# jkrasting/momlevel

Hardware: AMD Instinct MI355X
Metric: Mcells/s for fused Wright-EOS+steric at 1440×1080×75; % HBM roofline (higher is better)
Workload: dtype f64

## Files before the change

momlevel_amd/core.py:

```python

import numpy as np
import torch

from . import _lib, hostio
from ._lib import (
    DTYPE_F32,
    DTYPE_F32_UPCAST,
    DTYPE_F64,
    DTYPE_T32_S64,
    DTYPE_T64_S32,
    EOS_IDS,
    FUNC_IDS,
    P_FULL3D,
    P_FULL4D,
    P_SCALAR,
    P_ZPROF,
    MomlevelHipError,
)

F32_MODES = {"faithful": DTYPE_F32, "upcast": DTYPE_F32_UPCAST}
K1_TCHUNK = {"steric": 32, "held": 64}
ARITH_FLAGS = {"exact": 0, "fused": _lib.FLAG_FMA}


def arith_default(kernel="k0", dtype=None):
    import os

    mode = os.environ.get("MOMLEVEL_AMD_ARITH")
    if mode is None:
        return "fused" if kernel == "k1" else "exact"
    if mode not in ARITH_FLAGS:
        raise ValueError(f"MOMLEVEL_AMD_ARITH must be 'exact' or 'fused', got '{mode}'")
    return mode


def _arith_flag(arith, kernel="k0", dtype=None):
    if dtype in (DTYPE_T32_S64, DTYPE_T64_S32):
        if arith == "fused":
            raise ValueError("arith='fused' is not available for thetao / so of different dtypes")
        return 0
    if arith is None:
        arith = arith_default(kernel, dtype)
    try:
        return ARITH_FLAGS[arith]
    except KeyError:
        raise ValueError(f"arith must be 'exact' or 'fused', got '{arith}'") from None


def require_device():
    _lib.load()
    if not torch.cuda.is_available():
        raise MomlevelHipError(
            "no HIP device visible: momlevel_amd computes on MI355X only (no CPU fallback)"
        )
# ... 116 lines not shown
    while p.dim() > 3 and p.shape[0] == 1:
        p = p[0]
    shape = tuple(p.shape)
    if shape in ((nz,), (nz, 1, 1)):
        return p.reshape(nz), P_ZPROF
    if shape == (nz, ny, nx):
        return p, P_FULL3D
    if allow4d and shape == (nt, nz, ny, nx):
        return p, P_FULL4D
    try:
        return p.expand(nz, ny, nx).contiguous(), P_FULL3D
    except RuntimeError:
        pass
    if allow4d:
        return p.expand(nt, nz, ny, nx).contiguous(), P_FULL4D
    raise ValueError(f"pressure of shape {shape} does not broadcast to {(nz, ny, nx)}")


K0_PATHS = {_lib.PATH_GENERIC: "generic", _lib.PATH_FAST: "fast", _lib.PATH_FAST_P3D: "fast_p3d"}
PROMOTE_KINDS = {"d": _lib.KIND_F64, "f": _lib.KIND_F32, "w": _lib.KIND_WEAK}
_PROMOTE_FUNCS = {"inverse_barometer": _lib.FUNC_IBH, "density_ref": _lib.FUNC_DENSITY_REF}


def k0_path(dtype, p_mode, eos, func, plane, sT, sS, flags=0, aligned16=_lib.PATH_ALIGNED_ALL):
    import ctypes

    cells, steps = ctypes.c_int64(0), ctypes.c_int64(0)
    rc = _lib.load_path().mlx_path_eos_map(int(dtype), int(p_mode), int(eos), int(func), int(plane),
                                           int(sT), int(sS), int(flags), int(aligned16),
                                           ctypes.byref(cells), ctypes.byref(steps))
    if rc < 0:
        _lib.check(rc, "mlx_path_eos_map")
    return K0_PATHS[rc], int(cells.value), int(steps.value)


def promote_path(kinds, eos="wright", func="density", aligned16=_lib.PATH_ALIGNED_ALL):
    import ctypes

    kind = ctypes.c_int(-1)
    fid = _PROMOTE_FUNCS.get(func)
    if fid is None:
        fid = FUNC_IDS[func]
    rc = _lib.load_path().mlx_path_eos_promote(*(PROMOTE_KINDS[k] for k in kinds),
                                               EOS_IDS[eos.lower()], fid, int(aligned16),
                                               ctypes.byref(kind))
    if rc < 0:
        _lib.check(rc, "mlx_path_eos_promote")
    return rc, (torch.float32 if kind.value == _lib.KIND_F32 else torch.float64)


def _is16(t):
    return t is not None and t.data_ptr() % 16 == 0


def _k0_call(T, S, p, eos, f32_mode, flags_of, out):
    T, S, nt, nz, ny, nx, sT, sS, dt, squeeze = _pair(T, S, f32_mode)
    pt, p_mode = _pressure(p, nt, nz, ny, nx, T.device, allow4d=True)
    if dt in (DTYPE_T32_S64, DTYPE_T64_S32):
        return T, S, dt, pt, p_mode, EOS_IDS[eos.lower()], nt, nz, ny * nx, sT, sS, 0, out, squeeze
    if out is not None and squeeze and out.dim() == 3:
        out = out.unsqueeze(0)
    out = _out_like(out, (nt, nz, ny, nx), torch.float64, T.device, "float64")
    return (T, S, dt, pt, p_mode, EOS_IDS[eos.lower()], nt, nz, ny * nx, sT, sS, flags_of(dt), out,
            squeeze)


# ... 1119 lines not shown
```

momlevel_amd/csrc/momlevel_hip.hip:

```cpp

#include <hip/hip_runtime.h>
#include <stdint.h>
#include <stdio.h>
#include <string.h>

#include <initializer_list>
#include <type_traits>

#include "../../include/momlevel_hip.h"
#include "eos_device.hpp"
#include "mlx_internal.hpp"

#pragma clang fp contract(off)

namespace mlx {

constexpr int kBlock = 256;
constexpr int kNTC = 8;

template <typename TIn, int VEC>
struct Pack {
  TIn v[VEC];
};

// ... 76 lines not shown
__device__ __forceinline__ void store_pack(float* __restrict__ p, const Pack<float, VEC>& r) {
  if constexpr (VEC == 1) {
    if constexpr (STREAM) __builtin_nontemporal_store(r.v[0], p);
    else p[0] = r.v[0];
  } else if constexpr (VEC == 2) {
    double raw;
    __builtin_memcpy(&raw, &r, 8);
    if constexpr (STREAM) __builtin_nontemporal_store(raw, reinterpret_cast<double*>(p));
    else *reinterpret_cast<double*>(p) = raw;
  } else {
    static_assert(VEC == 4, "float packs are 4, 8 or 16 bytes");
    f4_t raw;
    __builtin_memcpy(&raw, &r, 16);
    if constexpr (STREAM) __builtin_nontemporal_store(raw, reinterpret_cast<f4_t*>(p));
    else *reinterpret_cast<f4_t*>(p) = raw;
  }
}

__device__ __forceinline__ void lds_dma16(const void* gsrc, void* lds_slice) {
#if defined(__HIP_DEVICE_COMPILE__)
  __builtin_amdgcn_global_load_lds(gsrc, (__attribute__((address_space(3))) void*)lds_slice, 16, 0,
                                   2 );
#endif
}

__device__ __forceinline__ double wave_sum(double v) {
#pragma unroll
  for (int off = 32; off > 0; off >>= 1) v += __shfl_down(v, off, 64);
  return v;
}

constexpr int kVarSteric = 0, kVarHalo = 1, kVarThermo = 2, kVarAll = 3;

template <typename TIn, int VEC, int U, int VAR, int MODE, bool GENERIC, bool SKIP, bool FMA,
          bool P3D = false>
__global__ __launch_bounds__(kBlock) void k_steric_global(
    const TIn* __restrict__ T, const TIn* __restrict__ S, const TIn* __restrict__ T0,
    const TIn* __restrict__ S0, const double* __restrict__ vol0, const double* __restrict__ p,
    int p_mode, int eos, int nt, int t_chunk, int64_t plane, int64_t t_stride_T,
    int64_t t_stride_S, double* __restrict__ partials, int64_t nblk_total) {
  constexpr int NOUT = (VAR == kVarAll) ? 4 : 1;
  constexpr int NTC = (VAR == kVarAll) ? kNTC / 2 : kNTC;
  constexpr bool STREAM_T = (VAR != kVarHalo), STREAM_S = (VAR != kVarThermo);
  constexpr bool HELD_T = (VAR == kVarHalo || VAR == kVarAll);
  constexpr bool HELD_S = (VAR == kVarThermo || VAR == kVarAll);
  typedef typename PolyType<MODE>::type R;
  typedef typename PolyVec<MODE, GENERIC ? 1 : VEC>::type RV;
  constexpr int W = Lanes<RV>::n, G = VEC / W;
  constexpr bool GUARD = !GENERIC && VAR != kVarAll;
  constexpr bool PRED = !(VAR == kVarSteric && sizeof(TIn) == 8);
  typedef typename std::conditional<
      FMA, typename FusedFor<MODE>::type,
      typename std::conditional<GUARD, typename ExactFastFor<MODE>::type, ExactOps>::type>::type Ops;
  __shared__ double red[NOUT][NTC][kBlock];

  const int tid = threadIdx.x;
  const int z = blockIdx.y;
  const int nz = gridDim.y;
  const int tb = blockIdx.z * t_chunk;
  const int te = (tb + t_chunk < nt) ? (tb + t_chunk) : nt;
  const int64_t bx = xcd_remap(blockIdx.x, gridDim.x);
  const int64_t blk = (int64_t)blockIdx.y * gridDim.x + bx;
  const int64_t tile0 = bx * (kBlock * VEC * U);
  const int64_t zoff = (int64_t)z * plane;

  int64_t off[U];
  double vol[U][VEC];
  double pc[U][VEC];
  bool alive[U];
#pragma unroll
  for (int u = 0; u < U; ++u) {
    int64_t i = tile0 + ((int64_t)u * kBlock + tid) * VEC;
    const bool valid = (i + VEC <= plane);
    i = valid ? i : 0;
    off[u] = zoff + i;
    Pack<double, VEC> v = load_pack<double, VEC>(vol0 + off[u]);
    bool any_wet = false;
#pragma unroll
    for (int k = 0; k < VEC; ++k) {
      vol[u][k] = valid ? v.v[k] : canonical_nan();
      if constexpr (Ops::contracts && MLX_TUNE_FMA_ACC)
        vol[u][k] = (vol[u][k] == 0.0) ? canonical_nan() : vol[u][k];
      any_wet = any_wet || !is_nan(vol[u][k]);
    }
    alive[u] = !SKIP || any_wet;
    if ((GENERIC && p_mode == MLX_P_FULL3D) || P3D) {
      Pack<double, VEC> q = load_pack<double, VEC>(p + off[u]);
#pragma unroll
      for (int k = 0; k < VEC; ++k) pc[u][k] = q.v[k];
    }
  }
  static_assert(!(P3D && GENERIC), "P3D is the fast kernels' form of MLX_P_FULL3D");
  static_assert(!Ops::fused || W == 1, "pressure folding is per cell");
  double pz = 0.0;
  if ((!GENERIC && !P3D) || p_mode == MLX_P_ZPROF) pz = p[z];
// ... 741 lines not shown
  snprintf(g_err, sizeof(g_err), "%s", msg);
  return code;
}

int hip_status(hipError_t e, const char* what) {
  if (e == hipSuccess) return 0;
  snprintf(g_err, sizeof(g_err), "%s: %s", what, hipGetErrorString(e));
  return (int)e;
}

}

int mlx::detail::fail(int code, const char* msg) { return ::fail(code, msg); }
int mlx::detail::hip_status(hipError_t e, const char* what) { return ::hip_status(e, what); }

namespace {

inline bool aligned(const void* p, size_t a) { return (reinterpret_cast<uintptr_t>(p) % a) == 0; }

inline int64_t ceil_div(int64_t a, int64_t b) { return a / b + (a % b != 0); }

inline bool mul_fits(int64_t a, int64_t b, int64_t* out, int64_t limit = INT64_MAX / 16) {
  return !__builtin_mul_overflow(a, b, out) && *out >= 0 && *out <= limit;
}

inline bool extents_fit(int64_t nt, int64_t nz, int64_t plane) {
  int64_t n3, n4;
  return mul_fits(nz, plane, &n3) && mul_fits(nt, n3, &n4);
}

constexpr int kU64 = 4, kVec64 = 2;
constexpr int kU32 = 2, kVec32 = 4;
constexpr int kUGen = 4;
constexpr int kTChunk = 32;
constexpr int kTChunkHeld = 64;
constexpr int kNTIGen = 8;

#ifndef MLX_TUNE_NTI64
#define MLX_TUNE_NTI64 0
#endif
#ifndef MLX_TUNE_NTI32
#define MLX_TUNE_NTI32 0
#endif
#ifndef MLX_TUNE_K2_VEC32
#define MLX_TUNE_K2_VEC32 0
#endif
#ifndef MLX_TUNE_K2_TBMAJOR
#define MLX_TUNE_K2_TBMAJOR 1
#endif
constexpr int k2_vec32(int var, bool drho) {
  if (MLX_TUNE_K2_VEC32) return MLX_TUNE_K2_VEC32;
  return (var == kVarSteric && !drho) ? 4 : 2;
}
#ifndef MLX_TUNE_K2_VEC64
#define MLX_TUNE_K2_VEC64 0
#endif
constexpr int k2_vec64(int var, bool drho) {
  if (MLX_TUNE_K2_VEC64) return MLX_TUNE_K2_VEC64;
  return 2;
}
constexpr int k2_nti(bool f64, int var, bool drho) {
  if (f64 && MLX_TUNE_NTI64) return MLX_TUNE_NTI64;
  if (!f64 && MLX_TUNE_NTI32) return MLX_TUNE_NTI32;
  if (f64) return (var == kVarSteric) ? 16 : 8;
  if (var == kVarSteric && !drho) return 6;
  return drho ? 16 : 12;
}

constexpr int kKnownFlags = MLX_FLAG_SKIP_DRY | MLX_FLAG_FMA | MLX_FLAG_TCHUNK_MASK;
// ... 70 lines not shown
struct K0Path {
  int kind;
  int64_t cells_per_block;
};

K0Path k0_path(int dtype, int p_mode, int eos, int func, int64_t plane, int64_t sT, int64_t sS,
               int aligned16) {
  const int fields = path::kAlignedT | path::kAlignedS | path::kAlignedOut;
  const bool fast = fast_shape(dtype, p_mode, eos, plane, sT, sS, (aligned16 & fields) == fields,
                               func == MLX_FUNC_DENSITY && (aligned16 & path::kAlignedP)) &&
                    (dtype == MLX_DTYPE_F64 || func == MLX_FUNC_DENSITY) && func != MLX_FUNC_IBH;
  if (!fast) return K0Path{path::kGeneric, (int64_t)kBlock * kK0CellsGeneric};
  return K0Path{p_mode == MLX_P_FULL3D ? path::kFastP3D : path::kFast,
                (int64_t)kBlock * vec_of(dtype) * kK0PacksFast};
}

template <int V>
using Int = std::integral_constant<int, V>;
template <typename F>
auto with_dtype(int dtype, F&& f) {
  switch (dtype) {
    case MLX_DTYPE_F64: return f(double{}, Int<kF64>{});
    case MLX_DTYPE_F32: return f(float{}, Int<kF32Faithful>{});
    case MLX_DTYPE_T32_S64: return f(double{}, Int<kMixT32>{});
    case MLX_DTYPE_T64_S32: return f(double{}, Int<kMixS32>{});
    default: return f(float{}, Int<kF32Upcast>{});
  }
}

struct K1Args {
  hipStream_t st;
  const void *T, *S, *T0, *S0;
  const double *vol0, *p;
  int p_mode, eos, nt, nz, t_chunk;
  int64_t plane, sT, sS;
  double* partials;
  int64_t nblk;
  bool p3d;
};

template <typename TIn, int VEC, int U, int VAR, int MODE, bool GEN, bool SKIP, bool FMA,
          bool P3D>
int k1_launch(K1Args& a) {
  const int64_t gx = ceil_div(a.plane, (int64_t)kBlock * VEC * U), ntc = ceil_div(a.nt, a.t_chunk);
  if (ntc > 65535) return fail(MLX_E_SHAPE, "nt too large for one call: chunk it");
  if (gx > 2147483647LL) return fail(MLX_E_SHAPE, "plane too large");
  a.nblk = gx * a.nz;
  snprintf(g_kernel, sizeof(g_kernel), "k_steric_global<%s,%d,%d,%d,%d,%s,%s,%s%s>",
           type_name<TIn>(), VEC, U, VAR, MODE, tf(GEN), tf(SKIP), tf(FMA), P3D ? ",true" : "");
  hipLaunchKernelGGL((k_steric_global<TIn, VEC, U, VAR, MODE, GEN, SKIP, FMA, P3D>),
                     dim3((unsigned)gx, (unsigned)a.nz, (unsigned)ntc), dim3(kBlock), 0, a.st,
                     (const TIn*)a.T, (const TIn*)a.S, (const TIn*)a.T0, (const TIn*)a.S0, a.vol0,
                     a.p, a.p_mode, a.eos, a.nt, a.t_chunk, a.plane, a.sT, a.sS, a.partials, a.nblk);
  return 0;
}

template <typename TIn, int VEC, int U, int VAR, int MODE, bool GEN, bool SKIP, bool FMA>
int k1_go(K1Args& a) {
  if constexpr (!GEN && VAR != kVarAll) {
    if (a.p3d) return k1_launch<TIn, VEC, U, VAR, MODE, GEN, SKIP, FMA, true>(a);
  }
  return k1_launch<TIn, VEC, U, VAR, MODE, GEN, SKIP, FMA, false>(a);
}

template <typename TIn, int VEC, int U, int VAR, int MODE, bool GEN>
int k1_flags(K1Args& a, bool skip, bool fma) {
  constexpr bool S1 = !GEN;
  if constexpr (!IsMixed<MODE>::value) {
    if (fma)
      return (skip && S1) ? k1_go<TIn, VEC, U, VAR, MODE, GEN, S1, true>(a)
                          : k1_go<TIn, VEC, U, VAR, MODE, GEN, false, true>(a);
  }
  return (skip && S1) ? k1_go<TIn, VEC, U, VAR, MODE, GEN, S1, false>(a)
                      : k1_go<TIn, VEC, U, VAR, MODE, GEN, false, false>(a);
}

template <typename TIn, int VEC, int U, int MODE, bool GEN>
int k1_var(K1Args& a, int var, bool skip, bool fma) {
  if constexpr (GEN) {
    if (var == kVarAll) return k1_flags<TIn, VEC, U, kVarAll, MODE, GEN>(a, skip, fma);
    return k1_flags<TIn, VEC, U, kVarSteric, MODE, GEN>(a, skip, fma);
  } else {
    switch (var) {
      case kVarSteric: return k1_flags<TIn, VEC, U, kVarSteric, MODE, GEN>(a, skip, fma);
      case kVarHalo: return k1_flags<TIn, VEC, U, kVarHalo, MODE, GEN>(a, skip, fma);
      case kVarThermo: return k1_flags<TIn, VEC, U, kVarThermo, MODE, GEN>(a, skip, fma);
      default: return k1_flags<TIn, VEC, U, kVarAll, MODE, GEN>(a, skip, fma);
    }
  }
}

int k1_dispatch(K1Args& a, int dtype, bool fast, int var, bool skip, bool fma) {
  return with_dtype(dtype, [&](auto tin, auto mode) {
    using TIn = decltype(tin);
    constexpr int MODE = decltype(mode)::value;
    constexpr bool F64 = sizeof(TIn) == 8;
    if (fast)
      return k1_var<TIn, F64 ? kVec64 : kVec32, F64 ? kU64 : kU32, MODE, false>(a, var, skip, fma);
    return k1_var<TIn, 1, kUGen, MODE, true>(a, var, skip, fma);
  });
}

int k1_time_chunk(int flags, int64_t nt, int var) {
  const int hint = (flags & MLX_FLAG_TCHUNK_MASK) >> 8;
  int64_t tc = hint ? (int64_t)hint * 8 : (var == kVarSteric ? kTChunk : kTChunkHeld);
  if (tc > nt) tc = nt;
  return (int)tc;
}

int steric_global_impl(const void* T, const void* S, const void* T0, const void* S0, int var,
                       int dtype, const double* vol0, const double* p, int p_mode, int eos,
                       int64_t nt, int64_t nz, int64_t plane, int64_t sT, int64_t sS, int flags,
                       double* out, void* workspace, size_t workspace_bytes, void* stream,
                       const char* name) {
  const int nout = (var == kVarAll) ? 4 : 1;
  if (flags & ~kKnownFlags) return fail(MLX_E_ENUM, "unknown flag bits");
  if (int rc = check_common(T, S, dtype, p, p_mode, eos, nt, nz, plane, sT, sS, true)) return rc;
  if (mixed_dtype(dtype) && (flags & MLX_FLAG_FMA))
    return fail(MLX_E_ENUM, "MLX_FLAG_FMA is not available for theta/salinity of different dtypes");
  if (!vol0 || !out) return fail(MLX_E_NULL, "vol0 and the output must not be NULL");
  if (!aligned(vol0, 8) || !aligned(out, 8)) return fail(MLX_E_ALIGN, "vol0/out not 8-byte aligned");
  if (var == kVarAll) {
    if (!T0 || !S0) return fail(MLX_E_NULL, "T0 and S0 must not be NULL");
    if (!aligned(T0, elem_size(dtype, true)) || !aligned(S0, elem_size(dtype, false)))
      return fail(MLX_E_ALIGN, "T0/S0 not element-aligned");
  }
  if (!workspace) return fail(MLX_E_NULL, "workspace must not be NULL");
  const size_t need = (size_t)nout * mlx_steric_global_workspace_bytes(nt, nz, plane);
  if (!aligned(workspace, 8) || workspace_bytes < need)
    return fail(MLX_E_WORKSPACE, "workspace smaller than the *_workspace_bytes() query");
  const bool skip = (flags & MLX_FLAG_SKIP_DRY) != 0, fma = (flags & MLX_FLAG_FMA) != 0;
  bool fast = fast_layout(dtype, p_mode, eos, plane, sT, sS, {T, S, T0, S0, vol0},
                          var != kVarAll ? p : nullptr);
  if (var != kVarAll) {
    if (sT == 0 && sS == 0) fast = false;
    else if (sT == 0) { var = kVarHalo; T0 = T; }
    else if (sS == 0) { var = kVarThermo; S0 = S; }
  }
  K1Args a;
  a.p3d = fast && p_mode == MLX_P_FULL3D;
  a.t_chunk = k1_time_chunk(flags, nt, var);
  a.st = (hipStream_t)stream;
  a.T = T; a.S = S; a.T0 = T0 ? T0 : T; a.S0 = S0 ? S0 : S;
  a.vol0 = vol0; a.p = p ? p : vol0;
  a.p_mode = p_mode; a.eos = eos; a.nt = (int)nt; a.nz = (int)nz;
  a.plane = plane; a.sT = sT; a.sS = sS;
  a.partials = (double*)workspace;
  if (int rc = k1_dispatch(a, dtype, fast, var, skip, fma)) return rc;
  if (int rc = hip_status(hipGetLastError(), name)) return rc;
  hipLaunchKernelGGL(k_reduce_rows, dim3((unsigned)(nout * nt)), dim3(kBlock), 0, a.st,
                     a.partials, a.nblk, out);
  return hip_status(hipGetLastError(), "k_reduce_rows launch");
}

struct K2Args {
  hipStream_t st;
  const void *T, *S, *T0, *S0;
  const double *rho0m, *surf, *dz, *z_i, *deptho, *p;
  int p_mode, eos, nt, nz;
  double neg_inv_rhozero;
  int64_t plane, sT, sS;
  void* drho;
  double* eta;
  int64_t drho_vstride, eta_vstride;
  bool drho32;
  bool p3d;
};

template <typename TIn, int VEC, int NTI, int VAR, int MODE, bool GEN, bool SKIP, bool FMA,
          bool P3D, bool DRHO32 = false>
int k2_launch(const K2Args& a) {
  typedef typename std::conditional<DRHO32, float, double>::type TOut;
  const int64_t gx = ceil_div(a.plane, (int64_t)kBlock * VEC), ntb = ceil_div(a.nt, NTI);
  if (ntb > 65535) return fail(MLX_E_SHAPE, "nt too large for one call: chunk it");
// ... 262 lines not shown
                     int64_t* launch_steps) {
  if (flags & ~MLX_FLAG_FMA) return fail(MLX_E_ENUM, "mlx_eos_map takes MLX_FLAG_FMA only");
  if (int rc = check_dtype(dtype, false)) return rc;
  if (eos != MLX_EOS_WRIGHT && eos != MLX_EOS_LINEAR) return fail(MLX_E_ENUM, "unknown eos");
  if (p_mode < MLX_P_SCALAR || p_mode > MLX_P_FULL4D) return fail(MLX_E_ENUM, "unknown p_mode");
  if (func < MLX_FUNC_DENSITY || func > MLX_FUNC_IBH) return fail(MLX_E_ENUM, "unknown func");
  if ((flags & MLX_FLAG_FMA) && func != MLX_FUNC_DENSITY)
    return fail(MLX_E_ENUM, "MLX_FLAG_FMA applies to the density only");
  if (aligned16 & ~path::kAlignedAll) return fail(MLX_E_ENUM, "unknown bits in aligned16");
  if (plane <= 0) return fail(MLX_E_SHAPE, "plane must be > 0");
  if (plane > (int64_t)1 << 40) return fail(MLX_E_SHAPE, "plane too large");
  if (sT < 0 || sS < 0) return fail(MLX_E_SHAPE, "time strides must be >= 0");
  const K0Path route = k0_path(dtype, p_mode, eos, func, plane, sT, sS, aligned16);
  if (cells_per_block) *cells_per_block = route.cells_per_block;
  if (launch_steps) *launch_steps = kK0LaunchSteps;
  return route.kind;
}

int mlx_eos_map(const void* T, const void* S, int dtype, const double* p, int p_mode, int eos,
                int func, int64_t nt, int64_t nz, int64_t plane, int64_t sT, int64_t sS,
                int flags, double* out, void* stream) {
  if (func == MLX_FUNC_IBH) return fail(MLX_E_ENUM, "use mlx_inverse_barometer for MLX_FUNC_IBH");
  return eos_map_impl(T, S, dtype, p, p_mode, eos, func, 0.0, nt, nz, plane, sT, sS, flags, out,
                      stream);
}

int mlx_inverse_barometer(const void* T, const void* S, int dtype, const double* p, int p_mode,
                          int eos, double gravity, int64_t nt, int64_t nz, int64_t plane,
                          int64_t sT, int64_t sS, double* out, void* stream) {
  return eos_map_impl(T, S, dtype, p, p_mode, eos, MLX_FUNC_IBH, gravity, nt, nz, plane, sT, sS,
                      0, out, stream);
}

size_t mlx_steric_global_workspace_bytes(int64_t nt, int64_t nz, int64_t plane) {
  if (nt <= 0 || nz <= 0 || plane <= 0) return 0;
  int64_t nblk, n;
  if (!mul_fits(ceil_div(plane, (int64_t)kBlock * kUGen), nz, &nblk) || !mul_fits(nt, nblk, &n))
    return 0;
  return (size_t)n * sizeof(double);
}

size_t mlx_steric_global_decomp_workspace_bytes(int64_t nt, int64_t nz, int64_t plane) {
  return 4 * mlx_steric_global_workspace_bytes(nt, nz, plane);
}

int mlx_steric_global(const void* T, const void* S, int dtype, const double* vol0, const double* p,
                      int p_mode, int eos, int64_t nt, int64_t nz, int64_t plane, int64_t sT,
                      int64_t sS, int flags, double* masso_out, void* workspace,
                      size_t workspace_bytes, void* stream) {
  return steric_global_impl(T, S, nullptr, nullptr, kVarSteric, dtype, vol0, p, p_mode, eos, nt,
                            nz, plane, sT, sS, flags, masso_out, workspace, workspace_bytes,
                            stream, "k_steric_global launch");
}

int mlx_steric_global_decomp(const void* T, const void* S, const void* T0, const void* S0,
                             int dtype, const double* vol0, const double* p, int p_mode, int eos,
                             int64_t nt, int64_t nz, int64_t plane, int64_t sT, int64_t sS,
                             int flags, double* out, void* workspace, size_t workspace_bytes,
                             void* stream) {
  if (sT == 0 || sS == 0)
    return fail(MLX_E_SHAPE, "mlx_steric_global_decomp streams both fields: time strides must be > 0");
  return steric_global_impl(T, S, T0, S0, kVarAll, dtype, vol0, p, p_mode, eos, nt, nz, plane, sT,
                            sS, flags, out, workspace, workspace_bytes, stream,
                            "k_steric_global (decomposition) launch");
}

// ... 189 lines not shown
```

momlevel_amd/_lib.py:

```python

import ctypes
import os

HERE = os.path.dirname(os.path.abspath(__file__))
LIB_PATH = os.environ.get("MOMLEVEL_AMD_LIB") or os.path.join(HERE, "libmomlevel_hip.so")
_ORACLE_DIR = os.path.join(os.path.dirname(HERE), "oracle")

ABI_VERSION = 9
EOS_WRIGHT, EOS_LINEAR = 0, 1
FUNC_DENSITY, FUNC_DRHO_DTEMP, FUNC_DRHO_DSAL, FUNC_ALPHA, FUNC_BETA, FUNC_IBH = 0, 1, 2, 3, 4, 5
FUNC_DENSITY_REF = 6
P_SCALAR, P_ZPROF, P_FULL3D, P_FULL4D = 0, 1, 2, 3
DTYPE_F64, DTYPE_F32, DTYPE_F32_UPCAST = 0, 1, 2
DTYPE_T32_S64, DTYPE_T64_S32 = 3, 4
FLAG_SKIP_DRY = 1
FLAG_FMA = 2
FLAG_DRHO_F32 = 4
BUILD_HIP, BUILD_HOST = 1, 2
KIND_F64, KIND_F32, KIND_WEAK = 0, 1, 2
STRAT_N2, STRAT_TURNER = 0, 1
TREND_MAX_TERMS = 8
(APPLY_REMOVE, APPLY_CORRECT, APPLY_TREND, APPLY_TREND_ANOM, APPLY_MODEL_RESID,
 APPLY_MODEL) = range(6)
STAT_MEAN, STAT_STD, STAT_MIN, STAT_MAX = range(4)
GAUGE_ROW_X, GAUGE_ROW_Y, GAUGE_ROW_Z, GAUGE_ROW_PHI, GAUGE_ROW_LAM = range(5)
GAUGE_ROWS = 5
VORT_UNITS_M, VORT_UNITS_CM = 0, 1
VORT_TILE_LANES, VORT_TILE_H, VORT_TILE_BANDS = 64, 16, 4
AREA_MAX_SLOTS = 16
AREA_WINDOW = 32
LAYER_MAX = 8
FILTER_NORMALISE = 1
QUANTILE_MAX_Q = 8
PATH_GENERIC, PATH_FAST, PATH_FAST_P3D = 0, 1, 2
PATH_ALIGNED_T, PATH_ALIGNED_S, PATH_ALIGNED_OUT, PATH_ALIGNED_P = 1, 2, 4, 8
PATH_ALIGNED_ALL = 15


def flag_tchunk(steps):
    return ((int(steps) // 8) & 0xFF) << 8


EOS_IDS = {"wright": EOS_WRIGHT, "linear": EOS_LINEAR}
FUNC_IDS = {
    "density": FUNC_DENSITY,
    "drho_dtemp": FUNC_DRHO_DTEMP,
    "drho_dsal": FUNC_DRHO_DSAL,
    "alpha": FUNC_ALPHA,
    "beta": FUNC_BETA,
}

_vp = ctypes.c_void_p
_i64 = ctypes.c_int64
_int = ctypes.c_int
_dbl = ctypes.c_double
_sz = ctypes.c_size_t
_u64 = ctypes.c_uint64

SIGNATURES = {
    "mlx_version": (_int, []),
    "mlx_last_error": (_int, [ctypes.c_char_p, _sz]),
    "mlx_build_kind": (_int, []),
    "mlx_last_kernel": (_int, [ctypes.c_char_p, _sz]),
    "mlx_eos_map": (
        _int,
        [_vp, _vp, _int, _vp, _int, _int, _int, _i64, _i64, _i64, _i64, _i64, _int, _vp, _vp],
# ... 100 lines not shown

LAYER_SIGNATURES = {
    "mlx_layer_steps": (_int, []),
    "mlx_layer_record_blocks": (_int, [_i64]),
    "mlx_layer_integral": (_int, [_vp, _int, _i64, _i64, _i64, _vp, _vp, _vp, _vp, _int, _vp, _dbl,
                                  _vp, _vp]),
}


FILTER_SIGNATURES = {
    "mlx_filter_tile": (_i64, []),
    "mlx_filter_window_edge": (_i64, [_int]),
    "mlx_filter_tiles_per_block": (_i64, [_i64, _i64, _int]),
    "mlx_filter_apply": (_int, [_vp, _int, _vp, _i64, _i64, _i64, _i64, _int, _i64, _i64, _vp, _int,
                               _vp]),
}


QUANTILE_SIGNATURES = {
    "mlx_quantile_block_cells": (_i64, [_int]),
    "mlx_quantile_unroll": (_i64, []),
    "mlx_quantile_select": (_int, [_vp, _int, _vp, _vp, _i64, _i64, _i64, _i64, _vp, _int, _vp,
                                   _vp]),
    "mlx_quantile_exceed_count": (_int, [_vp, _int, _vp, _vp, _i64, _i64, _i64, _i64, _vp, _vp,
                                         _vp]),
}


PATH_SIGNATURES = {
    "mlx_path_eos_map": (_int, [_int, _int, _int, _int, _i64, _i64, _i64, _int, _int,
                                ctypes.POINTER(ctypes.c_int64), ctypes.POINTER(ctypes.c_int64)]),
    "mlx_path_eos_promote": (_int, [_int, _int, _int, _int, _int, _int,
                                    ctypes.POINTER(ctypes.c_int)]),
}


class MomlevelHipError(RuntimeError):
    """Raised when the HIP library is missing or one of its calls fails."""


def _declare(lib, table, rebuild_with=None):
    for name, (restype, argtypes) in table.items():
        try:
            fn = getattr(lib, name)
        except AttributeError as exc:
            hint = "" if rebuild_with is None else (
                f": rebuild it with {rebuild_with} (`python -m momlevel_amd.csrc.build --force`)")
            raise MomlevelHipError(f"{LIB_PATH} does not export {name}{hint}") from exc
        fn.restype = restype
        fn.argtypes = argtypes


_lib = None


def load():
    global _lib
    if _lib is not None:
        return _lib
    if not os.path.exists(LIB_PATH):
        raise MomlevelHipError(
            f"{LIB_PATH} not found: momlevel_amd has no CPU fallback. Build the HIP "
            "library with `python -m momlevel_amd.csrc.build` (needs hipcc)."
        )
    real = os.path.realpath(LIB_PATH)
    if os.path.commonpath([real, os.path.realpath(_ORACLE_DIR)]) == os.path.realpath(_ORACLE_DIR):
        raise MomlevelHipError(
            f"{LIB_PATH} is under oracle/ (the CPU checker): momlevel_amd binds the HIP library only"
        )
    try:
        lib = ctypes.CDLL(LIB_PATH)
    except OSError as exc:
        raise MomlevelHipError(f"cannot load {LIB_PATH}: {exc}") from exc
    _declare(lib, SIGNATURES)
    if lib.mlx_version() != ABI_VERSION:
        raise MomlevelHipError(
            f"ABI mismatch: library {lib.mlx_version()} vs binding {ABI_VERSION}; rebuild"
        )
    if lib.mlx_build_kind() != BUILD_HIP:
        raise MomlevelHipError(
            f"{LIB_PATH} is build kind {lib.mlx_build_kind()}, not the HIP build "
            f"({BUILD_HIP}): momlevel_amd has no CPU backend"
        )
    _lib = lib
    return lib


_GROUPS = {
    "trend": (TREND_SIGNATURES, "the trend kernels"),
    "clim": (CLIM_SIGNATURES, "the grouped-statistic kernel"),
    "gauge": (GAUGE_SIGNATURES, "the tide-gauge kernels"),
    "spice": (SPICE_SIGNATURES, "the spiciness kernel"),
    "vort": (VORT_SIGNATURES, "the vorticity kernels"),
    "area": (AREA_SIGNATURES, "the area-mean kernels"),
    "layer": (LAYER_SIGNATURES, "the layer-integral kernel"),
    "filter": (FILTER_SIGNATURES, "the time-filter kernel"),
    "path": (PATH_SIGNATURES, "the path queries of the EOS maps"),
    "quantile": (QUANTILE_SIGNATURES, "the quantile kernels"),
}


_trend_bound = _clim_bound = _gauge_bound = _spice_bound = _vort_bound = _area_bound = False
_layer_bound = _filter_bound = _path_bound = _quantile_bound = False


def _load_group(group):
    lib = load()
    flag = f"_{group}_bound"
    if not globals().get(flag, False):
        _declare(lib, *_GROUPS[group])
        globals()[flag] = True
    return lib


def load_trend():
    return _load_group("trend")


def load_clim():
    return _load_group("clim")


def load_gauge():
    return _load_group("gauge")


def load_spice():
    return _load_group("spice")


def load_vort():
    return _load_group("vort")


def load_area():
    return _load_group("area")


def load_layer():
    return _load_group("layer")


def load_filter():
    return _load_group("filter")


def load_path():
    return _load_group("path")


def load_quantile():
    return _load_group("quantile")


def last_error():
    buf = ctypes.create_string_buffer(512)
    load().mlx_last_error(buf, 512)
    return buf.value.decode(errors="replace")


def last_kernel():
    buf = ctypes.create_string_buffer(160)
    load().mlx_last_kernel(buf, 160)
    return buf.value.decode(errors="replace")


def check(status, what):
    if status != 0:
        kind = "argument error" if status < 0 else "hipError_t"
        raise MomlevelHipError(f"{what} failed: {kind} {status}: {last_error()}")
```

momlevel_amd/csrc/build.py:

```python

import os
import shutil
import subprocess
import sys

HERE = os.path.dirname(os.path.abspath(__file__))
PKG = os.path.dirname(HERE)
ROOT = os.path.dirname(PKG)
_TIMED_UNITS = ["momlevel_hip.hip", "momlevel_promote.hip"]
FEATURES = {
    "strat": ["eos_device.hpp", "mlx_internal.hpp", "mlx_pack.hpp"],
    "trend": ["eos_device.hpp", "mlx_internal.hpp", "mlx_pack.hpp", "mlx_record.hpp",
              "include/momlevel_trend.h"],
    "clim": ["eos_device.hpp", "mlx_internal.hpp", "mlx_pack.hpp", "mlx_record.hpp",
             "include/momlevel_clim.h"],
    "gauge": ["eos_device.hpp", "mlx_internal.hpp", "mlx_pack.hpp", "mlx_record.hpp",
              "include/momlevel_gauge.h"],
    "spice": ["mlx_internal.hpp", "mlx_pack.hpp", "include/momlevel_spice.h"],
    "vort": ["mlx_internal.hpp", "mlx_pack.hpp", "include/momlevel_vort.h"],
    "area": ["mlx_internal.hpp", "mlx_pack.hpp", "include/momlevel_area.h"],
    "layer": ["mlx_internal.hpp", "mlx_pack.hpp", "include/momlevel_layer.h"],
    "filter": ["eos_device.hpp", "mlx_internal.hpp", "mlx_pack.hpp", "mlx_record.hpp",
               "include/momlevel_filter.h"],
    "quantile": ["eos_device.hpp", "mlx_internal.hpp", "mlx_pack.hpp", "mlx_record.hpp",
# ... 4 lines not shown
def _path(name):
    return os.path.join(ROOT, name) if name.startswith("include/") else os.path.join(HERE, name)


def _feature_files(feature):
    return [_path(f"momlevel_{feature}.hip")] + [_path(name) for name in FEATURES[feature]]


SOURCES = [_path(name) for name in _TIMED_UNITS + [f"momlevel_{f}.hip" for f in FEATURES]
           + ["host_copy.cpp"]]
LIB = os.path.join(PKG, "libmomlevel_hip.so")

FLAGS = [
    "--offload-arch=gfx950",
    "-O3",
    "-ffp-contract=off",
    "-fPIC",
    "-shared",
    "-std=c++17",
    "-Wall",
    "-Wno-unused-variable",
    "-Wno-sometimes-uninitialized",
]


TIMED_SOURCES = [
    os.path.join(HERE, "momlevel_hip.hip"),
    os.path.join(HERE, "eos_device.hpp"),
    os.path.join(HERE, "mlx_internal.hpp"),
    os.path.join(HERE, "momlevel_promote.hip"),
    os.path.join(HERE, "eos_promote.hpp"),
    os.path.join(ROOT, "include", "momlevel_hip.h"),
    os.path.join(ROOT, "include", "momlevel_path.h"),
]
DEPENDS = sorted({*SOURCES, *TIMED_SOURCES, *(p for f in FEATURES for p in _feature_files(f)),
                  os.path.abspath(__file__)})


def source_sha(paths=None, flags=True):
    import hashlib

    h = hashlib.sha256()
    for path in (TIMED_SOURCES if paths is None else paths):
        with open(path, "rb") as f:
            h.update(f.read())
    if flags:
        h.update(" ".join(FLAGS).encode())
    return h.hexdigest()[:16]


def feature_source_sha(feature):
    return source_sha(_feature_files(feature))


def strat_source_sha():
    return feature_source_sha("strat")


def trend_source_sha():
    return feature_source_sha("trend")


def clim_source_sha():
    return feature_source_sha("clim")


# ... 61 lines not shown
```

Measured before the change: 386,400.

## Schedule f64 steric blocks in cohorts sharing tiles across time chunks

```diff
diff --git a/momlevel_amd/core.py b/momlevel_amd/core.py
--- a/momlevel_amd/core.py
+++ b/momlevel_amd/core.py
@@ -19,7 +19,8 @@
 )
 
 F32_MODES = {"faithful": DTYPE_F32, "upcast": DTYPE_F32_UPCAST}
-K1_TCHUNK = {"steric": 32, "held": 64}
+K1_TCHUNK = {"steric": 8, "held": 64}
+K1_COHORT = 512
 ARITH_FLAGS = {"exact": 0, "fused": _lib.FLAG_FMA}
 
 
diff --git a/momlevel_amd/csrc/momlevel_hip.hip b/momlevel_amd/csrc/momlevel_hip.hip
--- a/momlevel_amd/csrc/momlevel_hip.hip
+++ b/momlevel_amd/csrc/momlevel_hip.hip
@@ -132,13 +132,16 @@
 
 constexpr int kVarSteric = 0, kVarHalo = 1, kVarThermo = 2, kVarAll = 3;
 
+template <typename TIn, int VAR, int MODE, bool GENERIC>
+constexpr bool k1_cohorts = sizeof(TIn) == 8 && MODE == kF64 && VAR == kVarSteric && !GENERIC;
+
 template <typename TIn, int VEC, int U, int VAR, int MODE, bool GENERIC, bool SKIP, bool FMA,
           bool P3D = false>
 __global__ __launch_bounds__(kBlock) void k_steric_global(
     const TIn* __restrict__ T, const TIn* __restrict__ S, const TIn* __restrict__ T0,
     const TIn* __restrict__ S0, const double* __restrict__ vol0, const double* __restrict__ p,
     int p_mode, int eos, int nt, int t_chunk, int64_t plane, int64_t t_stride_T,
-    int64_t t_stride_S, double* __restrict__ partials, int64_t nblk_total) {
+    int64_t t_stride_S, double* __restrict__ partials, int64_t nblk_total, int cohort) {
   constexpr int NOUT = (VAR == kVarAll) ? 4 : 1;
   constexpr int NTC = (VAR == kVarAll) ? kNTC / 2 : kNTC;
   constexpr bool STREAM_T = (VAR != kVarHalo), STREAM_S = (VAR != kVarThermo);
@@ -155,12 +158,32 @@
   __shared__ double red[NOUT][NTC][kBlock];
 
   const int tid = threadIdx.x;
-  const int z = blockIdx.y;
+  int z = blockIdx.y;
   const int nz = gridDim.y;
-  const int tb = blockIdx.z * t_chunk;
+  int tb = blockIdx.z * t_chunk;
+  int64_t bx, blk;
+  if (k1_cohorts<TIn, VAR, MODE, GENERIC> && cohort > 0) {
+    const int n = (int)nblk_total, ntc = (nt + t_chunk - 1) / t_chunk;
+    const int gx = (int)((plane + (kBlock * VEC * U - 1)) / (kBlock * VEC * U));
+    const int nfull = n / cohort, per_cohort = cohort * ntc;
+    int c = (int)blockIdx.x / per_cohort, items = cohort, slots = cohort;
+    if (c >= nfull) {
+      c = nfull;
+      items = n - nfull * cohort;
+      slots = (items + 7) & ~7;
+    }
+    const int r = (int)blockIdx.x - c * per_cohort, w = r / slots, item = r - w * slots;
+    if (item >= items) return;
+    const int pos = c * cohort + (int)xcd_remap(item, items);
+    z = pos / gx;
+    bx = pos - z * gx;
+    blk = pos;
+    tb = w * t_chunk;
+  } else {
+    bx = xcd_remap(blockIdx.x, gridDim.x);
+    blk = (int64_t)blockIdx.y * gridDim.x + bx;
+  }
   const int te = (tb + t_chunk < nt) ? (tb + t_chunk) : nt;
-  const int64_t bx = xcd_remap(blockIdx.x, gridDim.x);
-  const int64_t blk = (int64_t)blockIdx.y * gridDim.x + bx;
   const int64_t tile0 = bx * (kBlock * VEC * U);
   const int64_t zoff = (int64_t)z * plane;
 
@@ -968,7 +991,13 @@
 constexpr int kU64 = 4, kVec64 = 2;
 constexpr int kU32 = 2, kVec32 = 4;
 constexpr int kUGen = 4;
-constexpr int kTChunk = 32;
+constexpr int kTChunk = 8;
+constexpr int kTChunkPlain = 32;
+#ifndef MLX_TUNE_K1_COHORT
+#define MLX_TUNE_K1_COHORT 512
+#endif
+constexpr int kK1Cohort = MLX_TUNE_K1_COHORT;
+static_assert(kK1Cohort >= 0 && kK1Cohort % 8 == 0, "a cohort is a whole number of XCD rounds");
 constexpr int kTChunkHeld = 64;
 constexpr int kNTIGen = 8;
 
@@ -1123,10 +1152,20 @@
   a.nblk = gx * a.nz;
   snprintf(g_kernel, sizeof(g_kernel), "k_steric_global<%s,%d,%d,%d,%d,%s,%s,%s%s>",
            type_name<TIn>(), VEC, U, VAR, MODE, tf(GEN), tf(SKIP), tf(FMA), P3D ? ",true" : "");
-  hipLaunchKernelGGL((k_steric_global<TIn, VEC, U, VAR, MODE, GEN, SKIP, FMA, P3D>),
-                     dim3((unsigned)gx, (unsigned)a.nz, (unsigned)ntc), dim3(kBlock), 0, a.st,
-                     (const TIn*)a.T, (const TIn*)a.S, (const TIn*)a.T0, (const TIn*)a.S0, a.vol0,
-                     a.p, a.p_mode, a.eos, a.nt, a.t_chunk, a.plane, a.sT, a.sS, a.partials, a.nblk);
+  dim3 grid((unsigned)gx, (unsigned)a.nz, (unsigned)ntc);
+  int cohort = 0;
+  if constexpr (k1_cohorts<TIn, VAR, MODE, GEN> && kK1Cohort > 0) {
+    const int64_t rag = a.nblk % kK1Cohort;
+    const int64_t blocks = ntc * (a.nblk - rag + (rag + 7) / 8 * 8);
+    if (ntc > 1 && blocks <= kK2MaxBlocks1D) {
+      cohort = kK1Cohort;
+      grid = dim3((unsigned)blocks);
+    }
+  }
+  hipLaunchKernelGGL((k_steric_global<TIn, VEC, U, VAR, MODE, GEN, SKIP, FMA, P3D>), grid,
+                     dim3(kBlock), 0, a.st, (const TIn*)a.T, (const TIn*)a.S, (const TIn*)a.T0,
+                     (const TIn*)a.S0, a.vol0, a.p, a.p_mode, a.eos, a.nt, a.t_chunk, a.plane,
+                     a.sT, a.sS, a.partials, a.nblk, cohort);
   return 0;
 }
 
@@ -1176,9 +1215,10 @@
   });
 }
 
-int k1_time_chunk(int flags, int64_t nt, int var) {
+int k1_time_chunk(int flags, int64_t nt, int var, bool cohorts) {
   const int hint = (flags & MLX_FLAG_TCHUNK_MASK) >> 8;
-  int64_t tc = hint ? (int64_t)hint * 8 : (var == kVarSteric ? kTChunk : kTChunkHeld);
+  const int steric = (cohorts && kK1Cohort > 0) ? kTChunk : kTChunkPlain;
+  int64_t tc = hint ? (int64_t)hint * 8 : (var == kVarSteric ? steric : kTChunkHeld);
   if (tc > nt) tc = nt;
   return (int)tc;
 }
@@ -1214,7 +1254,7 @@
   }
   K1Args a;
   a.p3d = fast && p_mode == MLX_P_FULL3D;
-  a.t_chunk = k1_time_chunk(flags, nt, var);
+  a.t_chunk = k1_time_chunk(flags, nt, var, fast && dtype == MLX_DTYPE_F64);
   a.st = (hipStream_t)stream;
   a.T = T; a.S = S; a.T0 = T0 ? T0 : T; a.S0 = S0 ? S0 : S;
   a.vol0 = vol0; a.p = p ? p : vol0;
```

Measured after the change: 392,700, median of 5. 1.02x the previous value.

## Balance K1 time windows into equal parking-group splits and raise steric chunk

Applied to the files above, without the earlier changes.

```diff
diff --git a/include/momlevel_window.h b/include/momlevel_window.h
--- /dev/null
+++ b/include/momlevel_window.h
@@ -0,0 +1,22 @@
+#ifndef MOMLEVEL_WINDOW_H
+#define MOMLEVEL_WINDOW_H
+
+#include <stddef.h>
+#include <stdint.h>
+
+#ifdef __cplusplus
+extern "C" {
+#endif
+
+#define MLX_WINDOW_STERIC 0
+#define MLX_WINDOW_HALO   1
+#define MLX_WINDOW_THERMO 2
+#define MLX_WINDOW_ALL    3
+
+int mlx_window_k1(int dtype, int variant, int flags, int64_t nt, int *steps, int *n_short,
+                  int *depth);
+
+#ifdef __cplusplus
+}
+#endif
+#endif
diff --git a/momlevel_amd/_lib.py b/momlevel_amd/_lib.py
--- a/momlevel_amd/_lib.py
+++ b/momlevel_amd/_lib.py
@@ -32,6 +32,7 @@
 LAYER_MAX = 8
 FILTER_NORMALISE = 1
 QUANTILE_MAX_Q = 8
+WINDOW_STERIC, WINDOW_HALO, WINDOW_THERMO, WINDOW_ALL = range(4)
 PATH_GENERIC, PATH_FAST, PATH_FAST_P3D = 0, 1, 2
 PATH_ALIGNED_T, PATH_ALIGNED_S, PATH_ALIGNED_OUT, PATH_ALIGNED_P = 1, 2, 4, 8
 PATH_ALIGNED_ALL = 15
@@ -198,6 +199,12 @@
                                 ctypes.POINTER(ctypes.c_int64), ctypes.POINTER(ctypes.c_int64)]),
     "mlx_path_eos_promote": (_int, [_int, _int, _int, _int, _int, _int,
                                     ctypes.POINTER(ctypes.c_int)]),
+}
+
+
+WINDOW_SIGNATURES = {
+    "mlx_window_k1": (_int, [_int, _int, _int, _i64, ctypes.POINTER(ctypes.c_int),
+                             ctypes.POINTER(ctypes.c_int), ctypes.POINTER(ctypes.c_int)]),
 }
 
 
@@ -263,6 +270,7 @@
     "filter": (FILTER_SIGNATURES, "the time-filter kernel"),
     "path": (PATH_SIGNATURES, "the path queries of the EOS maps"),
     "quantile": (QUANTILE_SIGNATURES, "the quantile kernels"),
+    "window": (WINDOW_SIGNATURES, "the time-window query of the K1 launches"),
 }
 
 
@@ -319,6 +327,10 @@
     return _load_group("quantile")
 
 
+def load_window():
+    return _load_group("window")
+
+
 def last_error():
     buf = ctypes.create_string_buffer(512)
     load().mlx_last_error(buf, 512)
diff --git a/momlevel_amd/core.py b/momlevel_amd/core.py
--- a/momlevel_amd/core.py
+++ b/momlevel_amd/core.py
@@ -19,7 +19,7 @@
 )
 
 F32_MODES = {"faithful": DTYPE_F32, "upcast": DTYPE_F32_UPCAST}
-K1_TCHUNK = {"steric": 32, "held": 64}
+K1_TCHUNK = {"steric": 64, "steric_f32": 32, "held": 64, "long": 152}
 ARITH_FLAGS = {"exact": 0, "fused": _lib.FLAG_FMA}
 
 
@@ -202,6 +202,24 @@
     if rc < 0:
         _lib.check(rc, "mlx_path_eos_map")
     return K0_PATHS[rc], int(cells.value), int(steps.value)
+
+
+K1_VARIANTS = {"steric": _lib.WINDOW_STERIC, "halosteric": _lib.WINDOW_HALO,
+               "thermosteric": _lib.WINDOW_THERMO, "all": _lib.WINDOW_ALL}
+
+
+def k1_windows(nt, variant="steric", dtype=DTYPE_F64, skip_dry=False, t_chunk=0):
+    import ctypes
+
+    steps, n_short, depth = ctypes.c_int(0), ctypes.c_int(0), ctypes.c_int(0)
+    flags = (_lib.FLAG_SKIP_DRY if skip_dry else 0) | (_lib.flag_tchunk(t_chunk) if t_chunk else 0)
+    count = _lib.load_window().mlx_window_k1(int(dtype), K1_VARIANTS[variant], flags, int(nt),
+                                             ctypes.byref(steps), ctypes.byref(n_short),
+                                             ctypes.byref(depth))
+    if count < 0:
+        _lib.check(count, "mlx_window_k1")
+    starts = [i * steps.value + max(0, i - n_short.value) * depth.value for i in range(count)]
+    return [b - a for a, b in zip(starts, starts[1:] + [int(nt)])], depth.value
 
 
 def promote_path(kinds, eos="wright", func="density", aligned16=_lib.PATH_ALIGNED_ALL):
diff --git a/momlevel_amd/csrc/build.py b/momlevel_amd/csrc/build.py
--- a/momlevel_amd/csrc/build.py
+++ b/momlevel_amd/csrc/build.py
@@ -60,6 +60,7 @@
     os.path.join(HERE, "eos_promote.hpp"),
     os.path.join(ROOT, "include", "momlevel_hip.h"),
     os.path.join(ROOT, "include", "momlevel_path.h"),
+    os.path.join(ROOT, "include", "momlevel_window.h"),
 ]
 DEPENDS = sorted({*SOURCES, *TIMED_SOURCES, *(p for f in FEATURES for p in _feature_files(f)),
                   os.path.abspath(__file__)})
diff --git a/momlevel_amd/csrc/momlevel_hip.hip b/momlevel_amd/csrc/momlevel_hip.hip
--- a/momlevel_amd/csrc/momlevel_hip.hip
+++ b/momlevel_amd/csrc/momlevel_hip.hip
@@ -137,7 +137,7 @@
 __global__ __launch_bounds__(kBlock) void k_steric_global(
     const TIn* __restrict__ T, const TIn* __restrict__ S, const TIn* __restrict__ T0,
     const TIn* __restrict__ S0, const double* __restrict__ vol0, const double* __restrict__ p,
-    int p_mode, int eos, int nt, int t_chunk, int64_t plane, int64_t t_stride_T,
+    int p_mode, int eos, int nt, int t_chunk, int n_short, int64_t plane, int64_t t_stride_T,
     int64_t t_stride_S, double* __restrict__ partials, int64_t nblk_total) {
   constexpr int NOUT = (VAR == kVarAll) ? 4 : 1;
   constexpr int NTC = (VAR == kVarAll) ? kNTC / 2 : kNTC;
@@ -157,8 +157,10 @@
   const int tid = threadIdx.x;
   const int z = blockIdx.y;
   const int nz = gridDim.y;
-  const int tb = blockIdx.z * t_chunk;
-  const int te = (tb + t_chunk < nt) ? (tb + t_chunk) : nt;
+  const int wz = blockIdx.z;
+  const int tb = wz * t_chunk + (wz > n_short ? wz - n_short : 0) * NTC;
+  const int tlen = t_chunk + (wz >= n_short ? NTC : 0);
+  const int te = (tb + tlen < nt) ? (tb + tlen) : nt;
   const int64_t bx = xcd_remap(blockIdx.x, gridDim.x);
   const int64_t blk = (int64_t)blockIdx.y * gridDim.x + bx;
   const int64_t tile0 = bx * (kBlock * VEC * U);
@@ -968,9 +970,50 @@
 constexpr int kU64 = 4, kVec64 = 2;
 constexpr int kU32 = 2, kVec32 = 4;
 constexpr int kUGen = 4;
-constexpr int kTChunk = 32;
+constexpr int kNTIGen = 8;
+
+constexpr int kTChunk = 64;
+constexpr int kTChunk32 = 32;
 constexpr int kTChunkHeld = 64;
-constexpr int kNTIGen = 8;
+constexpr int kTChunkLong = 152;
+constexpr int k1_depth(int var) { return var == kVarAll ? kNTC / 2 : kNTC; }
+constexpr bool k1_equal_windows(bool f32, int var, bool skip) {
+  return !f32 && !(var == kVarThermo && !skip);
+}
+constexpr int k1_window_cap(bool f32, int var, bool skip) {
+  if (var == kVarSteric) return f32 ? kTChunk32 : kTChunk;
+  return k1_equal_windows(f32, var, skip) ? kTChunkLong : kTChunkHeld;
+}
+static_assert(kTChunk % kNTC == 0 && kTChunk32 % kNTC == 0 && kTChunkHeld % kNTC == 0 &&
+              kTChunkLong % kNTC == 0, "a cap is whole parking groups");
+
+struct K1Windows {
+  int base, n_short, count;
+};
+inline int64_t k1_window_start(const K1Windows& w, int64_t i, int depth) {
+  return i * w.base + (i > w.n_short ? i - w.n_short : 0) * depth;
+}
+inline K1Windows k1_fixed_windows(int64_t steps, int64_t nt) {
+  K1Windows w;
+  w.base = (int)(steps < nt ? steps : nt);
+  w.count = (int)ceil_div(nt, (int64_t)w.base);
+  w.n_short = w.count;
+  return w;
+}
+inline K1Windows k1_windows(int flags, int64_t nt, int var, bool f32) {
+  const bool skip = (flags & MLX_FLAG_SKIP_DRY) != 0;
+  const int hint = (flags & MLX_FLAG_TCHUNK_MASK) >> 8;
+  if (hint) return k1_fixed_windows((int64_t)hint * 8, nt);
+  const int64_t cap = k1_window_cap(f32, var, skip);
+  if (!k1_equal_windows(f32, var, skip)) return k1_fixed_windows(cap, nt);
+  const int64_t depth = k1_depth(var), groups = ceil_div(nt, depth);
+  const int64_t count = ceil_div(groups, cap / depth);
+  K1Windows w;
+  w.base = (int)(groups / count * depth);
+  w.count = (int)count;
+  w.n_short = (int)(count - groups % count);
+  return w;
+}
 
 #ifndef MLX_TUNE_NTI64
 #define MLX_TUNE_NTI64 0
@@ -1107,7 +1150,8 @@
   hipStream_t st;
   const void *T, *S, *T0, *S0;
   const double *vol0, *p;
-  int p_mode, eos, nt, nz, t_chunk;
+  int p_mode, eos, nt, nz;
+  K1Windows win;
   int64_t plane, sT, sS;
   double* partials;
   int64_t nblk;
@@ -1117,8 +1161,11 @@
 template <typename TIn, int VEC, int U, int VAR, int MODE, bool GEN, bool SKIP, bool FMA,
           bool P3D>
 int k1_launch(K1Args& a) {
-  const int64_t gx = ceil_div(a.plane, (int64_t)kBlock * VEC * U), ntc = ceil_div(a.nt, a.t_chunk);
+  const int64_t gx = ceil_div(a.plane, (int64_t)kBlock * VEC * U), ntc = a.win.count;
+  static_assert(k1_depth(VAR) == ((VAR == kVarAll) ? kNTC / 2 : kNTC), "the kernel's NTC");
   if (ntc > 65535) return fail(MLX_E_SHAPE, "nt too large for one call: chunk it");
+  if (k1_window_start(a.win, ntc - 1, k1_depth(VAR)) >= a.nt)
+    return fail(MLX_E_SHAPE, "internal: a time window starts past the record");
   if (gx > 2147483647LL) return fail(MLX_E_SHAPE, "plane too large");
   a.nblk = gx * a.nz;
   snprintf(g_kernel, sizeof(g_kernel), "k_steric_global<%s,%d,%d,%d,%d,%s,%s,%s%s>",
@@ -1126,7 +1173,8 @@
   hipLaunchKernelGGL((k_steric_global<TIn, VEC, U, VAR, MODE, GEN, SKIP, FMA, P3D>),
                      dim3((unsigned)gx, (unsigned)a.nz, (unsigned)ntc), dim3(kBlock), 0, a.st,
                      (const TIn*)a.T, (const TIn*)a.S, (const TIn*)a.T0, (const TIn*)a.S0, a.vol0,
-                     a.p, a.p_mode, a.eos, a.nt, a.t_chunk, a.plane, a.sT, a.sS, a.partials, a.nblk);
+                     a.p, a.p_mode, a.eos, a.nt, a.win.base, a.win.n_short, a.plane, a.sT, a.sS,
+                     a.partials, a.nblk);
   return 0;
 }
 
@@ -1176,11 +1224,8 @@
   });
 }
 
-int k1_time_chunk(int flags, int64_t nt, int var) {
-  const int hint = (flags & MLX_FLAG_TCHUNK_MASK) >> 8;
-  int64_t tc = hint ? (int64_t)hint * 8 : (var == kVarSteric ? kTChunk : kTChunkHeld);
-  if (tc > nt) tc = nt;
-  return (int)tc;
+inline bool k1_f32_caps(int dtype) {
+  return dtype == MLX_DTYPE_F32 || dtype == MLX_DTYPE_F32_UPCAST;
 }
 
 int steric_global_impl(const void* T, const void* S, const void* T0, const void* S0, int var,
@@ -1214,7 +1259,7 @@
   }
   K1Args a;
   a.p3d = fast && p_mode == MLX_P_FULL3D;
-  a.t_chunk = k1_time_chunk(flags, nt, var);
+  a.win = k1_windows(flags, nt, var, k1_f32_caps(dtype));
   a.st = (hipStream_t)stream;
   a.T = T; a.S = S; a.T0 = T0 ? T0 : T; a.S0 = S0 ? S0 : S;
   a.vol0 = vol0; a.p = p ? p : vol0;
@@ -1543,6 +1588,22 @@
                       0, out, stream);
 }
 
+int mlx_window_k1(int dtype, int variant, int flags, int64_t nt, int* steps, int* n_short,
+                  int* depth) {
+  static_assert(kVarSteric == 0 && kVarHalo == 1 && kVarThermo == 2 && kVarAll == 3,
+                "MLX_WINDOW_* of include/momlevel_window.h");
+  if (flags & ~kKnownFlags) return fail(MLX_E_ENUM, "unknown flag bits");
+  if (int rc = check_dtype(dtype, true)) return rc;
+  if (variant < kVarSteric || variant > kVarAll) return fail(MLX_E_ENUM, "unknown variant");
+  if (nt <= 0 || nt > 2147483647LL) return fail(MLX_E_SHAPE, "nt must be in 1 .. 2^31 - 1");
+  const K1Windows w = k1_windows(flags, nt, variant, k1_f32_caps(dtype));
+  if (w.count > 65535) return fail(MLX_E_SHAPE, "nt too large for one call: chunk it");
+  if (steps) *steps = w.base;
+  if (n_short) *n_short = w.n_short;
+  if (depth) *depth = k1_depth(variant);
+  return w.count;
+}
+
 size_t mlx_steric_global_workspace_bytes(int64_t nt, int64_t nz, int64_t plane) {
   if (nt <= 0 || nz <= 0 || plane <= 0) return 0;
   int64_t nblk, n;
```

After: 392,000 before, 387,400 after. -1.2%, worse.
